# 0xSooki/stark-rs

Measured on AMD Instinct MI355X. Metric: ntt_field_elements_per_sec, higher is better.
Workload: dtype u32; 1 GPU; lde_2^22rows_x4cols_blowup8 (4 iNTT 2^22 + 4 coset NTT 2^25 per GPU per step); prime=469762049, parallelism=columns x1 (no collective)

## Files before the change

### stark_rs_amd/csrc/emu.cpp

```cpp
#include <array>
#include <vector>

#include "ntt_driver.h"
#include "lde_core.h"
#include "tables.h"
#include "proof_parse.h"

namespace {

std::vector<uint32_t> fill(const GeomSpec &s, const Fp &F) {
    std::vector<uint32_t> t((size_t)s.count << s.pair);
    for (uint32_t i = 0; i < s.count; i++) {
        const uint32_t v = geom_entry(s.c_m, s.q_m, i, s.stride, F);
        if (s.pair) { const Tw2 c = tw2_from_mont(v, F); t[2 * i] = c.w; t[2 * i + 1] = c.q; }
        else t[i] = v;
    }
    return t;
}

template <int LOGR, int LOGW, int KIND, int CAP> void emu_pass_cols(const PassArgs &a) {
    typedef NttPass<LOGR, LOGW, KIND, CAP> NP;
    constexpr bool LAST = KIND == PASS_LAST;
    const uint32_t NT = NP::NT;
    std::vector<uint32_t> tile(NP::R * NP::WP);
    std::vector<Tw2> tw(NP::R);
    std::vector<std::array<uint32_t, 16>> mw(NT), mq(NT), iw(NT), regs(NT);
    const bool twin = KIND == PASS_MID && (a.flags & NTT_TW_IN);
    auto r16 = [](std::array<uint32_t, 16> &x) -> uint32_t(&)[16] { return reinterpret_cast<uint32_t(&)[16]>(x); };
    for (uint32_t blk = 0; blk < a.n_tiles; blk++) {
        typename NP::TileId t = NP::tile_id(a, blk);
        for (uint32_t tid = 0; tid < NT; tid++) NP::load_tw(a, tw.data(), tid);
        for (uint32_t b = 0; b < a.batch; b++) {
            if (b % NP::COLS_PER_WG == 0)
                for (uint32_t tid = 0; tid < NT; tid++) {
                    NP::out_mul(a, t, tid, r16(mw[tid]), r16(mq[tid]));
                    if (twin) NP::in_mul(a, t, tid, r16(iw[tid]));
                }
            if (twin) {
                for (uint32_t tid = 0; tid < NT; tid++) {
                    NP::template load_regs<0, false>(a, t, b, r16(regs[tid]), tid);
                    for (int i = 0; i < 16; i++) regs[tid][i] = mont_mul(regs[tid][i], iw[tid][i], a.F);
                }
                for (uint32_t tid = 0; tid < NT; tid++) NP::template step0_regs<0>(a, r16(regs[tid]), tile.data(), tw.data(), tid);
            } else if (!LAST) {
#define ZCASE(Z)                                                                                                 \
    case Z:                                                                                                      \
        for (uint32_t tid = 0; tid < NT; tid++) NP::template load_regs<Z>(a, t, b, r16(regs[tid]), tid);         \
        for (uint32_t tid = 0; tid < NT; tid++) NP::template step0_regs<Z>(a, r16(regs[tid]), tile.data(), tw.data(), tid); \
        break;
                switch (a.zlog) { ZCASE(2) ZCASE(3) ZCASE(4) default: ZCASE(0) }
#undef ZCASE
            } else if (a.flags & NTT_LAST_DIRECT) {
                for (uint32_t tid = 0; tid < NT; tid++) NP::load_rows_direct(a, t, b, r16(regs[tid]), tid);
                for (uint32_t tid = 0; tid < NT; tid++) NP::step0_rows(a, r16(regs[tid]), tile.data(), tw.data(), tid);
            } else {
                for (uint32_t tid = 0; tid < NT; tid++) NP::load_rows(a, t, b, r16(regs[tid]), tid);
                for (uint32_t tid = 0; tid < NT; tid++) NP::rows_to_lds(r16(regs[tid]), tile.data(), tid);
                for (uint32_t tid = 0; tid < NT; tid++) NP::step0_lds(a, tile.data(), tw.data(), tid);
// ... 4 lines not shown
    }
}

int g_share_cols = 1;

template <int LOGR, int LOGW, int KIND, int CAP> void emu_pass(const PassArgs &a, uint32_t batch) {
    typedef NttPass<LOGR, LOGW, KIND, CAP> NP;
    constexpr bool LAST = KIND == PASS_LAST;
    if (g_share_cols && NP::share_cols(a, g_share_cols == 2 ? 0u : (uint32_t)NP::COLS_MIN_WGS)) return emu_pass_cols<LOGR, LOGW, KIND, CAP>(a);
    std::vector<uint32_t> tile(NP::R * NP::WP);
    std::vector<Tw2> tw(NP::R);
    for (uint32_t b = 0; b < batch; b++)
        for (uint32_t blk = 0; blk < a.n_tiles; blk++) {
            typename NP::TileId t = NP::tile_id(a, blk);
            const uint32_t NT = NP::NT;
            for (uint32_t tid = 0; tid < NT; tid++) NP::load_tw(a, tw.data(), tid);
            if (!LAST) {
                std::vector<std::array<uint32_t, 16>> regs(NT);
#define ZCASE(Z)                                                                                                           \
    case Z:                                                                                                                \
        for (uint32_t tid = 0; tid < NT; tid++) NP::template load_regs<Z>(a, t, b, reinterpret_cast<uint32_t(&)[16]>(regs[tid]), tid); \
        for (uint32_t tid = 0; tid < NT; tid++) NP::template step0_regs<Z>(a, reinterpret_cast<uint32_t(&)[16]>(regs[tid]), tile.data(), tw.data(), tid); \
        break;
                switch (a.zlog) { ZCASE(0) ZCASE(1) ZCASE(2) ZCASE(3) ZCASE(4) }
#undef ZCASE
            } else if (a.flags & NTT_LAST_DIRECT) {
                std::vector<std::array<uint32_t, 16>> regs(NT);
                for (uint32_t tid = 0; tid < NT; tid++) NP::load_rows_direct(a, t, b, reinterpret_cast<uint32_t(&)[16]>(regs[tid]), tid);
                for (uint32_t tid = 0; tid < NT; tid++) NP::step0_rows(a, reinterpret_cast<uint32_t(&)[16]>(regs[tid]), tile.data(), tw.data(), tid);
            } else {
// ... 578 lines not shown
```

### stark_rs_amd/csrc/internal.h

```cpp
#pragma once
#include <string.h>
#include <hip/hip_runtime.h>

#include <stdlib.h>

#include <string>
#include <vector>

#include "../../include/stark_mi.h"
#include "fri_plan.h"
#include "tables.h"
#include "transcript_core.h"

struct ScaleEntry {
    uint32_t c, q, L;
    uint32_t *lo, *hi;
    uint64_t epoch;
};

struct ProfRec {
    const char *name;
    hipEvent_t e0, e1;
    double bytes;
    double mixes;
// ... 12 lines not shown
    uint32_t *d_root_tab[32] = {};
    uint32_t *scratch = nullptr;
    size_t scratch_elems = 0;
    void *tmp[4] = {nullptr, nullptr, nullptr, nullptr};
    size_t tmp_bytes[4] = {0, 0, 0, 0};
    int *d_flag = nullptr;
    void *pin[2] = {nullptr, nullptr};
    hipEvent_t pin_ev[2] = {nullptr, nullptr};
    void *pin_out = nullptr;
    size_t pin_out_bytes = 0;
    std::string err;
    bool prof_on = false;
    char prof_only[56] = {0};
    bool copy_probe = false;
    bool ntt_share_cols = !(getenv("SMI_NTT_SHARE_COLS") && atoi(getenv("SMI_NTT_SHARE_COLS")) == 0);
    bool ntt_twin_regs = !(getenv("SMI_NTT_TWIN_REGS") && atoi(getenv("SMI_NTT_TWIN_REGS")) == 0);
    bool ntt_last_direct = !(getenv("SMI_NTT_LAST_DIRECT") && atoi(getenv("SMI_NTT_LAST_DIRECT")) == 0);
    int ntt_defer_tw = getenv("SMI_NTT_DEFER_TW") ? (atoi(getenv("SMI_NTT_DEFER_TW")) != 0) : 2;
    bool lde_two_pass = getenv("SMI_LDE_TWO_PASS") && atoi(getenv("SMI_LDE_TWO_PASS"));
    std::vector<ProfRec> prof;
    uint8_t *arena = nullptr;
    size_t arena_size = 0, arena_used = 0, arena_want = 0;
    std::vector<void *> arena_overflow;
};
int arena_reset(smi_ctx *ctx);
void *arena_alloc(smi_ctx *ctx, size_t bytes);

struct ProfScope {
    smi_ctx *ctx;
    ProfRec r;
    bool on;
// ... 211 lines not shown
```

### stark_rs_amd/csrc/ntt.hip

```cpp
#include "internal.h"
#include "ntt_driver.h"
#include "lde_core.h"

template <int LOGR, int LOGW, int KIND, int CAP>
__global__ __launch_bounds__(1 << (LOGR + LOGW - 4)) void ntt_pass_kernel(const PassArgs a) {
    typedef NttPass<LOGR, LOGW, KIND, CAP> NP;
    __shared__ uint32_t tile[NP::R * NP::WP];
    __shared__ Tw2 tw[NP::R];
    const uint32_t tid = threadIdx.x, batch = blockIdx.y;
    const typename NP::TileId t = NP::tile_id(a, blockIdx.x);
    NP::load_tw(a, tw, tid);
    uint32_t v[NP::V];
    if constexpr (KIND == PASS_FIRST) {
#define ZCASE(Z)                                         \
    case Z:                                              \
        NP::template load_regs<Z>(a, t, batch, v, tid);  \
        __syncthreads();       \
        NP::template step0_regs<Z>(a, v, tile, tw, tid); \
        break;
        switch (a.zlog) { ZCASE(2) ZCASE(3) ZCASE(4) default: ZCASE(0) }
#undef ZCASE
    } else if constexpr (KIND == PASS_MID) {
        NP::template load_regs<0>(a, t, batch, v, tid);
        __syncthreads();
        NP::template step0_regs<0>(a, v, tile, tw, tid);
    } else if (a.flags & NTT_LAST_DIRECT) {
        NP::load_rows_direct(a, t, batch, v, tid);
// ... 7 lines not shown
    }
    __syncthreads();
    if (NP::St::n == 3) {
        NP::step_mid(a, tile, tw, tid);
        __syncthreads();
    }
    NP::last_step_store(a, t, batch, tile, tw, tid);
}

#ifndef SMI_COLS_WAVES
#define SMI_COLS_WAVES(TILE_LOG, LOGR) ((TILE_LOG) >= 14 || (LOGR) >= 11 ? 4 : ((LOGR) == 10 ? 5 : 6))
#endif
#ifndef SMI_COLS_TWIN_WAVES
#define SMI_COLS_TWIN_WAVES 4
#endif
#ifndef SMI_COLS_TWIN_MQ
#define SMI_COLS_TWIN_MQ 1
#endif
#ifndef SMI_COLS_PREFETCH
#define SMI_COLS_PREFETCH 1
#endif
template <int LOGR, int LOGW, int KIND, int CAP, bool TWIN = false>
__global__ __launch_bounds__(1 << (LOGR + LOGW - 4), TWIN ? SMI_COLS_TWIN_WAVES : SMI_COLS_WAVES(LOGR + LOGW, LOGR)) void ntt_pass_cols_kernel(const PassArgs a) {
    typedef NttPass<LOGR, LOGW, KIND, CAP> NP;
    __shared__ uint32_t tile[NP::R * NP::WP];
    __shared__ Tw2 tw[NP::R];
    const uint32_t tid0 = threadIdx.x;
    const typename NP::TileId t = NP::tile_id(a, blockIdx.x);
    NP::load_tw(a, tw, tid0);
    constexpr bool MQ = !TWIN || SMI_COLS_TWIN_MQ;
    uint32_t mw[NP::V], mq[MQ ? NP::V : 1];
    NP::template out_mul<MQ>(a, t, tid0, mw, mq);
    uint32_t iw[TWIN ? NP::V : 1];
    if constexpr (TWIN) NP::in_mul(a, t, tid0, iw);
    const uint32_t col0 = blockIdx.y * NP::COLS_PER_WG, col1 = min(a.batch, col0 + (uint32_t)NP::COLS_PER_WG);
    if constexpr (SMI_COLS_PREFETCH && KIND == PASS_MID && LOGW == 5) {
        uint32_t v[NP::V];
        auto load = [&](uint32_t col) {
            uint32_t tid = tid0;
            asm volatile("" : "+v"(tid));
            NP::template load_regs<0, !TWIN>(a, t, col, v, tid);
        };
        load(col0);
        for (uint32_t batch = col0; batch < col1; batch++) {
            uint32_t tid = tid0;
            asm volatile("" : "+v"(tid));
            if constexpr (TWIN) {
#pragma unroll
                for (int i = 0; i < NP::V; i++) v[i] = mont_mul(v[i], iw[i], a.F);
            }
            __syncthreads();
            NP::template step0_regs<0>(a, v, tile, tw, tid);
            if (batch + 1 < col1) load(batch + 1);
            __syncthreads();
            if (NP::St::n == 3) {
                NP::step_mid(a, tile, tw, tid);
                __syncthreads();
            }
            NP::template last_step_store_mul<MQ>(a, t, batch, tile, tw, tid, mw, mq);
        }
        return;
    }
    for (uint32_t batch = col0; batch < col1; batch++) {
        uint32_t tid = tid0;
        asm volatile("" : "+v"(tid));
        uint32_t v[NP::V];
        static_assert(KIND != PASS_FIRST, "first passes keep one workgroup per (tile, column), NttPass::share_cols");
        if constexpr (KIND == PASS_MID) {
            NP::template load_regs<0, !TWIN>(a, t, batch, v, tid);
            if constexpr (TWIN) {
#pragma unroll
                for (int i = 0; i < NP::V; i++) v[i] = mont_mul(v[i], iw[i], a.F);
            }
            __syncthreads();
            NP::template step0_regs<0>(a, v, tile, tw, tid);
        } else if (a.flags & NTT_LAST_DIRECT) {
            NP::load_rows_direct(a, t, batch, v, tid);
            __syncthreads();
            NP::step0_rows(a, v, tile, tw, tid);
        } else {
            NP::load_rows(a, t, batch, v, tid);
            if (batch != col0) __syncthreads();
            NP::rows_to_lds(v, tile, tid);
            __syncthreads();
            NP::step0_lds(a, tile, tw, tid);
        }
        __syncthreads();
        if (NP::St::n == 3) {
            NP::step_mid(a, tile, tw, tid);
            __syncthreads();
        }
        NP::template last_step_store_mul<MQ>(a, t, batch, tile, tw, tid, mw, mq);
    }
}

template <int LOGR, int LOGW, int KIND>
__global__ __launch_bounds__(1 << (LOGR + LOGW - 4)) void ntt_copy_probe_kernel(const PassArgs a) {
    typedef NttPass<LOGR, LOGW, KIND, 4> NP;
    enum { NB = (NP::TILE / NP::RL) / NP::NT, KSTEP_LOG = LOGR - NP::SL };
    const uint32_t tid = threadIdx.x, batch = blockIdx.y;
    const typename NP::TileId t = NP::tile_id(a, blockIdx.x);
    uint32_t v[NP::V];
    const uint32_t lin = a.flags >> 30;
    const uint64_t lin_in = (uint64_t)batch * a.in_stride + (uint64_t)blockIdx.x * NP::TILE;
    const uint64_t lin_out = (uint64_t)batch * a.out_stride + (uint64_t)blockIdx.x * NP::TILE;
    if ((lin & 1u) && KIND != PASS_FIRST) {
#pragma unroll
        for (int i = 0; i < NP::V; i++) v[i] = ld32(a.in + lin_in, (uint32_t)i * NP::NT + tid);
    } else if constexpr (KIND == PASS_LAST) {
        if (a.flags & NTT_LAST_DIRECT) NP::load_rows_direct(a, t, batch, v, tid);
        else NP::load_rows(a, t, batch, v, tid);
    } else if constexpr (KIND == PASS_MID) {
        NP::template load_regs<0, false>(a, t, batch, v, tid);
    } else {
        switch (a.zlog) {
        case 2: NP::template load_regs<2>(a, t, batch, v, tid); break;
        case 3: NP::template load_regs<3>(a, t, batch, v, tid); break;
        case 4: NP::template load_regs<4>(a, t, batch, v, tid); break;
        default: NP::template load_regs<0>(a, t, batch, v, tid); break;
        }
    }
    if ((lin & 2u) && KIND != PASS_LAST) {
#pragma unroll
        for (int i = 0; i < NP::V; i++) st32(a.out + lin_out, (uint32_t)i * NP::NT + tid, v[i] + 1u);
        return;
    }
    uint32_t *out = a.out + (uint64_t)batch * a.out_stride + t.out_base;
    const uint32_t sh = KIND == PASS_LAST ? a.Sp : a.L - a.Sp - LOGR;
// ... 123 lines not shown
    widen_kernel<<<grid_for(n, 256), 256, 0, ctx->stream>>>(d_in, d_out, n);
    HIP_TRY(ctx, hipGetLastError());
    return SMI_OK;
}

namespace {
struct HipLauncher {
    smi_ctx *ctx;
    hipError_t err = hipSuccess;
    void small(const SmallArgs &a, uint32_t batch) {
        ProfScope ps(ctx, "ntt_small_kernel", (4.0 * a.n_in + 4.0 * (1ull << a.L)) * batch);
        ntt_small_kernel<<<batch, SMI_NTT_THREADS, 0, ctx->stream>>>(a);
        note();
    }
    template <int LR, int LW, int KIND, int CAP> void launch(const PassArgs &a) {
        if constexpr (KIND != PASS_FIRST) {
            if (ctx->ntt_share_cols && NttPass<LR, LW, KIND, CAP>::share_cols(a)) {
                const dim3 grid(a.n_tiles, NttPass<LR, LW, KIND, CAP>::col_groups(a));
                if (KIND == PASS_MID && (a.flags & NTT_TW_IN) && ctx->ntt_twin_regs)
                    ntt_pass_cols_kernel<LR, LW, KIND, CAP, KIND == PASS_MID><<<grid, 1 << (LR + LW - 4), 0, ctx->stream>>>(a);
                else
                    ntt_pass_cols_kernel<LR, LW, KIND, CAP><<<grid, 1 << (LR + LW - 4), 0, ctx->stream>>>(a);
                return;
            }
        }
        ntt_pass_kernel<LR, LW, KIND, CAP><<<dim3(a.n_tiles, a.batch), 1 << (LR + LW - 4), 0, ctx->stream>>>(a);
    }
    template <int LR, int LW> void launch_probe(int kind, const PassArgs &a0) {
        static const uint32_t lin = getenv("SMI_PROBE_LINEAR") ? (uint32_t)atoi(getenv("SMI_PROBE_LINEAR")) & 3u : 0u;
        PassArgs a = a0;
        a.flags |= lin << 30;
        const dim3 grid(a.n_tiles, a.batch);
        if (kind == PASS_FIRST) ntt_copy_probe_kernel<LR, LW, PASS_FIRST><<<grid, 1 << (LR + LW - 4), 0, ctx->stream>>>(a);
        else if (kind == PASS_MID) ntt_copy_probe_kernel<LR, LW, PASS_MID><<<grid, 1 << (LR + LW - 4), 0, ctx->stream>>>(a);
        else ntt_copy_probe_kernel<LR, LW, PASS_LAST><<<grid, 1 << (LR + LW - 4), 0, ctx->stream>>>(a);
    }
    template <int LR, int LW, int CAP> void launch_kind(int kind, const PassArgs &a) {
        if (kind == PASS_FIRST) launch<LR, LW, PASS_FIRST, CAP>(a);
        else if (kind == PASS_MID) launch<LR, LW, PASS_MID, CAP>(a);
        else launch<LR, LW, PASS_LAST, CAP>(a);
    }
// ... 186 lines not shown
```

### stark_rs_amd/csrc/ntt_core.h

```cpp
#pragma once
#include "field.h"

#if defined(SMI_EMU_CHECKS) && !defined(__HIP_DEVICE_COMPILE__)
#include <assert.h>
#define SMI_BOUND_CHECK(x, m, p) assert((m) <= 8 && (uint64_t)(x) < (uint64_t)((m) ? (m) : 1) * (p) && ((m) || (x) == 0))
#else
#define SMI_BOUND_CHECK(x, m, p) ((void)0)
#endif

#define SMI_TILE_LOG 12
#define SMI_TILE (1u << SMI_TILE_LOG)
#define SMI_NTT_THREADS 256
#define SMI_TW_LOG 12

struct alignas(8) Tw2 {
    uint32_t w, q;
};

struct NttTables {
    const Tw2 *tw10;
    const uint32_t *lo;
    const uint32_t *hi;
    uint32_t K, h;
};
// ... 68 lines not shown
#if defined(SMI_NTT_DBG_NOSTORE)
    if (v != 0xFFFFFFFFu) return;
#endif
#if defined(__HIP_DEVICE_COMPILE__) && SMI_NTT_NT
    __builtin_nontemporal_store(v, p);
#else
    *p = v;
#endif
}
SMI_HD Tw2 ld_tw(const Tw2 *base, uint32_t idx) { return *(const Tw2 *)((const char *)base + (size_t)(uint32_t)(idx << 3)); }

SMI_HD uint32_t shoup_mul(uint32_t a, const Tw2 &c, uint32_t p) {
    return a * c.w - umulhi32(a, c.q) * p;
}
SMI_HD uint32_t lz_canon(uint32_t a, uint32_t p) { return umin32(a, a - p); }

SMI_HD void lz_fold_m(uint32_t &x, int &m, uint32_t p) {
    if (m > 4) { x = umin32(x, x - 4u * p); m = 4; }
    else if (m > 2) { x = umin32(x, x - 2u * p); m = 2; }
}
SMI_HD void lz_fold_to2(uint32_t &x, int &m, uint32_t p) {
    lz_fold_m(x, m, p);
    lz_fold_m(x, m, p);
}
SMI_HD uint32_t lz_canon_m(uint32_t x, int m, uint32_t p) {
    lz_fold_to2(x, m, p);
    return m > 1 ? umin32(x, x - p) : x;
}

template <int S, int CAP, int Z = 0>
// ... 15 lines not shown
#pragma unroll
            for (int t = 0; t < 3; t++)
                if (m[i] + m[j] > CAP) {
                    if (m[i] >= m[j]) lz_fold_m(x[i], m[i], p);
                    else lz_fold_m(x[j], m[j], p);
                }
            const uint32_t u = x[i], v = x[j];
            const int ms = m[i] + m[j];
            SMI_BOUND_CHECK(u, m[i], p);
            SMI_BOUND_CHECK(v, m[j], p);
            x[i] = u + v;
            const uint32_t d = u - v + (uint32_t)m[j] * p;
            m[i] = ms;
            if (e) { x[j] = shoup_mul(d, cw[e << croot_shift], p); m[j] = 2; }
            else { x[j] = d; m[j] = ms; }
        }
    }
}

enum { PASS_FIRST = 0, PASS_MID = 1, PASS_LAST = 2 };
template <int LOGR, int LOGW, int KIND, int CAP> struct NttPass {
    static constexpr bool FIRST = KIND == PASS_FIRST, MID = KIND == PASS_MID, LAST = KIND == PASS_LAST;
    enum { TILE_LOG = LOGR + LOGW, TILE = 1 << TILE_LOG, NT = TILE / 16, R = 1 << LOGR, W = 1 << LOGW, WP = W + 1, V = 16 };
    typedef Steps<LOGR> St;
    enum { SL = St::n == 2 ? St::s1 : St::s2, RL = 1 << SL };

    struct TileId {
        uint64_t in_base, out_base;
        uint32_t b0;
    };
// ... 22 lines not shown
            t.b0 = k0_0;
            t.in_base = (((uint64_t)k0_0 << arest_log) + a_rest) << LOGR;
            t.out_base = ((uint64_t)rev << a.d0_log) + k0_0;
        }
        return t;
    }

    static SMI_HD void load_tw(const PassArgs &a, Tw2 *tw, uint32_t tid) {
#pragma unroll
        for (int i = 0; i < (R + NT - 1) / NT; i++) {
            uint32_t j = tid + i * NT;
            if (j < (uint32_t)R) tw[j] = a.T.tw10[j << (SMI_TW_LOG - LOGR)];
        }
    }

    template <int Z, bool TWIN = true> static SMI_HD void load_regs(const PassArgs &a, const TileId &t, uint32_t batch, uint32_t (&v)[V], uint32_t tid) {
        const uint32_t blog = a.L - a.Sp - LOGR, ablog = blog - a.shard_log;
        const uint32_t w = tid & (W - 1), j0 = tid >> LOGW;
        const uint32_t o0 = (j0 << ablog) + w;
        if constexpr (FIRST) {
            const uint32_t *col = a.in + (uint64_t)batch * a.in_stride;
            const uint32_t n0 = a.b_off + t.b0 + (j0 << blog) + w;
#pragma unroll
            for (int i = 0; i < V; i++) {
                if (i >= (V >> Z)) { v[i] = 0u; continue; }
                const uint32_t g = n0 + ((uint32_t)(i * (NT >> LOGW)) << blog);
                const uint32_t ga = t.b0 + o0 + ((uint32_t)(i * (NT >> LOGW)) << ablog);
                const uint32_t x = ld32(col, g < a.n_in ? ga : 0u);
                v[i] = g < a.n_in ? x : 0u;
            }
            if (a.flags & NTT_PRE_SCALE) {
                uint32_t sc = two_level(a.S.lo, a.S.hi, a.S.h, n0, a.F);
                const uint32_t rq = a.pre_ratio_m * a.F.pinv;
#pragma unroll
                for (int i = 0; i < (V >> Z); i++) {
                    v[i] = mont_mul(v[i], sc, a.F);
                    sc = mont_mul_c(sc, a.pre_ratio_m, rq, a.F);
                }
            }
        } else {
            const uint32_t *in = a.in + (uint64_t)batch * a.in_stride + t.in_base;
#pragma unroll
            for (int i = 0; i < V; i++) v[i] = ld32(in, o0 + ((uint32_t)(i * (NT >> LOGW)) << ablog));
            if (TWIN && (a.flags & NTT_TW_IN)) {
                const uint32_t sub = (uint32_t)(t.in_base >> (a.L - a.Sp)), k = sub & ((1u << a.prev_logr) - 1u);
                const uint32_t sh = a.T.K - (a.L - a.Sp + a.prev_logr);
                uint32_t cur = two_level(a.T.lo, a.T.hi, a.T.h, (k * ((j0 << blog) + t.b0 + w)) << sh, a.F);
                const uint32_t ratio = two_level(a.T.lo, a.T.hi, a.T.h, (k * ((uint32_t)(NT >> LOGW) << blog)) << sh, a.F);
                const uint32_t rq = ratio * a.F.pinv;
#pragma unroll
                for (int i = 0; i < V; i++) {
                    v[i] = mont_mul(v[i], cur, a.F);
                    if (i + 1 < V) cur = mont_mul_c(cur, ratio, rq, a.F);
                }
            }
        }
    }

    template <int Z> static SMI_HD void step0_regs(const PassArgs &a, uint32_t (&x)[V], uint32_t *tile, const Tw2 *tw, uint32_t tid) {
        enum { SUB = LOGR - 4 };
        const uint32_t w = tid & (W - 1), pos = tid >> LOGW;
        int m[16];
#pragma unroll
        for (int i = 0; i < 16; i++) m[i] = i < (V >> Z) ? 1 : 0;
        dft_regs<4, CAP, Z>(x, m, tw, LOGR - 4, a.F);
#pragma unroll
        for (int kk = 0; kk < 16; kk++) {
            uint32_t v = x[brev<4>(kk)];
            int mv = m[brev<4>(kk)];
            if (kk) v = shoup_mul(v, tw[(pos * kk) & (R - 1)], a.F.p);
            else lz_fold_to2(v, mv, a.F.p);
// ... 42 lines not shown
        direct_map(tid, pos, line);
        int m[16];
#pragma unroll
        for (int i = 0; i < 16; i++) m[i] = 1;
        dft_regs<4, CAP>(x, m, tw, LOGR - 4, a.F);
#pragma unroll
        for (int kk = 0; kk < 16; kk++) {
            uint32_t v = x[brev<4>(kk)];
            int mv = m[brev<4>(kk)];
            if (kk) v = shoup_mul(v, tw[(pos * kk) & (R - 1)], a.F.p);
            else lz_fold_to2(v, mv, a.F.p);
            tile[(pos + ((uint32_t)kk << SUB)) * WP + line] = v;
        }
    }

    template <int S, int MLOG, int MIN> static SMI_HD void step(const PassArgs &a, uint32_t *tile, const Tw2 *tw, uint32_t tid) {
        enum { r = 1 << S, SUB = MLOG - S, NB = (TILE / r) / NT };
#pragma unroll
        for (int bi = 0; bi < NB; bi++) {
            const uint32_t u = tid + bi * NT;
            const uint32_t w = u & (W - 1), ub = u >> LOGW;
            const uint32_t blk = ub >> SUB, pos = ub & ((1u << SUB) - 1u);
            const uint32_t base = (blk << MLOG) + pos;
            uint32_t x[r];
#pragma unroll
            for (int q = 0; q < r; q++) x[q] = tile[(base + ((uint32_t)q << SUB)) * WP + w];
            int m[r];
#pragma unroll
            for (int q = 0; q < r; q++) m[q] = MIN;
            dft_regs<S, CAP>(x, m, tw, LOGR - S, a.F);
#pragma unroll
            for (int kk = 0; kk < r; kk++) {
                uint32_t v = x[brev<S>(kk)];
                int mv = m[brev<S>(kk)];
                if (kk) v = shoup_mul(v, tw[((pos * kk) << (LOGR - MLOG)) & (R - 1)], a.F.p);
                else lz_fold_to2(v, mv, a.F.p);
                tile[(base + ((uint32_t)kk << SUB)) * WP + w] = v;
            }
        }
    }
    static SMI_HD void step0_lds(const PassArgs &a, uint32_t *tile, const Tw2 *tw, uint32_t tid) { step<4, LOGR, 1>(a, tile, tw, tid); }
    static SMI_HD void step_mid(const PassArgs &a, uint32_t *tile, const Tw2 *tw, uint32_t tid) {
        if constexpr (St::n == 3) step<St::s1, LOGR - St::s0, 2>(a, tile, tw, tid);
    }

    static SMI_HD uint32_t blk_to_k(uint32_t blk) {
        if (St::n == 2) return blk;
        const uint32_t k0 = blk >> St::s1, k1 = blk & ((1u << St::s1) - 1u);
        return k0 | (k1 << St::s0);
    }

    static SMI_HD void last_step_store(const PassArgs &a, const TileId &t, uint32_t batch, const uint32_t *tile, const Tw2 *tw,
                                       uint32_t tid) {
        enum { NB = (TILE / RL) / NT, KSTEP_LOG = LOGR - SL };
        uint32_t *out = a.out + (uint64_t)batch * a.out_stride + t.out_base;
        const uint32_t mlog = a.L - a.Sp, p = a.F.p;
        uint32_t base_run = 0, gs = 0, gq = 0, gbi = 0, gbq = 0;
        uint32_t sc_run = 0, rq = 0, rbq = 0;
        if (!LAST && !(a.flags & NTT_TW_SKIP)) {
            const uint32_t b = a.b_off + t.b0 + (tid & (W - 1)), sh = a.T.K - mlog;
            base_run = two_level(a.T.lo, a.T.hi, a.T.h, (b * blk_to_k(tid >> LOGW)) << sh, a.F);
            gs = two_level(a.T.lo, a.T.hi, a.T.h, (b << KSTEP_LOG) << sh, a.F);
            gq = gs * a.F.pinv;
            if (NB > 1) {
                gbi = two_level(a.T.lo, a.T.hi, a.T.h, (b << SL) << sh, a.F);
                gbq = gbi * a.F.pinv;
            }
        }
        if (LAST && (a.flags & NTT_POST_SCALE)) {
            sc_run = two_level(a.S.lo, a.S.hi, a.S.h, (uint32_t)t.out_base + (blk_to_k(tid >> LOGW) << a.Sp) + (tid & (W - 1)), a.F);
            rq = a.post_ratio_m * a.F.pinv;
            rbq = a.post_bi_ratio_m * a.F.pinv;
        }
#pragma unroll
        for (int bi = 0; bi < NB; bi++) {
            const uint32_t u = tid + bi * NT;
            const uint32_t w = u & (W - 1), blk = u >> LOGW;
            uint32_t x[RL];
#pragma unroll
            for (int q = 0; q < RL; q++) x[q] = tile[(blk * RL + q) * WP + w];
            int m[RL];
#pragma unroll
            for (int q = 0; q < RL; q++) m[q] = 2;
            dft_regs<SL, CAP>(x, m, tw, LOGR - SL, a.F);
            const uint32_t kbase = blk_to_k(blk);
            if constexpr (!LAST) {
                const uint32_t blog = mlog - LOGR - a.shard_log;
                const uint32_t o0 = (kbase << blog) + w;
                {
                    if (a.flags & NTT_TW_SKIP) {
#pragma unroll
                        for (int kk = 0; kk < RL; kk++) {
                            SMI_BOUND_CHECK(x[brev<SL>(kk)], m[brev<SL>(kk)], p);
                            st32(out, o0 + ((uint32_t)kk << (KSTEP_LOG + blog)), x[brev<SL>(kk)]);
                        }
                        continue;
                    }
                    uint32_t cur = base_run;
                    if (bi + 1 < NB) base_run = mont_mul_c(base_run, gbi, gbq, a.F);
#pragma unroll
// ... 14 lines not shown
                    }
                } else {
#pragma unroll
                    for (int kk = 0; kk < RL; kk++) st32(out, o0 + ((uint32_t)kk << (KSTEP_LOG + a.Sp)), lz_canon_m(x[brev<SL>(kk)], m[brev<SL>(kk)], p));
                }
            }
        }
    }

    static SMI_HD bool has_out_mul(const PassArgs &a) { return LAST ? (a.flags & NTT_POST_SCALE) != 0 : !(a.flags & NTT_TW_SKIP); }
    enum { COLS_PER_WG = SMI_COLS_PER_WG, COLS_MIN_WGS = SMI_COLS_MIN_WGS };
    static SMI_HD uint32_t col_groups(const PassArgs &a) { return (a.batch + COLS_PER_WG - 1) / COLS_PER_WG; }
    static SMI_HD bool share_cols(const PassArgs &a, uint32_t min_wgs = COLS_MIN_WGS) {
        return !FIRST && a.batch > 1 && has_out_mul(a) && (uint64_t)a.n_tiles * col_groups(a) >= min_wgs;
    }
    template <bool MQ = true>
    static SMI_HD void out_mul(const PassArgs &a, const TileId &t, uint32_t tid, uint32_t (&mw)[V], uint32_t (&mq)[MQ ? V : 1]) {
        enum { NB = (TILE / RL) / NT, KSTEP_LOG = LOGR - SL };
        const uint32_t w = tid & (W - 1), kb0 = blk_to_k(tid >> LOGW);
        uint32_t run, step, step_bi = 0;
        if (!LAST) {
            const uint32_t b = a.b_off + t.b0 + w, sh = a.T.K - (a.L - a.Sp);
            run = two_level(a.T.lo, a.T.hi, a.T.h, (b * kb0) << sh, a.F);
            step = two_level(a.T.lo, a.T.hi, a.T.h, (b << KSTEP_LOG) << sh, a.F);
            if (NB > 1) step_bi = two_level(a.T.lo, a.T.hi, a.T.h, (b << SL) << sh, a.F);
        } else {
            run = two_level(a.S.lo, a.S.hi, a.S.h, (uint32_t)t.out_base + (kb0 << a.Sp) + w, a.F);
            step = a.post_ratio_m;
            step_bi = a.post_bi_ratio_m;
        }
        const uint32_t sq = step * a.F.pinv, bq = step_bi * a.F.pinv;
#pragma unroll
        for (int bi = 0; bi < NB; bi++) {
            uint32_t cur = run;
            if (bi + 1 < NB) run = mont_mul_c(run, step_bi, bq, a.F);
#pragma unroll
            for (int kk = 0; kk < RL; kk++) {
                mw[bi * RL + kk] = cur;
                if constexpr (MQ) mq[bi * RL + kk] = cur * a.F.pinv;
                if (kk + 1 < RL) cur = mont_mul_c(cur, step, sq, a.F);
            }
        }
    }
    static SMI_HD void in_mul(const PassArgs &a, const TileId &t, uint32_t tid, uint32_t (&iw)[V]) {
        const uint32_t blog = a.L - a.Sp - LOGR;
        const uint32_t w = tid & (W - 1), j0 = tid >> LOGW;
        const uint32_t sub = (uint32_t)(t.in_base >> (a.L - a.Sp)), k = sub & ((1u << a.prev_logr) - 1u);
        const uint32_t sh = a.T.K - (a.L - a.Sp + a.prev_logr);
        uint32_t cur = two_level(a.T.lo, a.T.hi, a.T.h, (k * ((j0 << blog) + t.b0 + w)) << sh, a.F);
        const uint32_t ratio = two_level(a.T.lo, a.T.hi, a.T.h, (k * ((uint32_t)(NT >> LOGW) << blog)) << sh, a.F);
        const uint32_t rq = ratio * a.F.pinv;
#pragma unroll
        for (int i = 0; i < V; i++) {
            iw[i] = cur;
            if (i + 1 < V) cur = mont_mul_c(cur, ratio, rq, a.F);
        }
    }
    template <bool MQ = true>
    static SMI_HD void last_step_store_mul(const PassArgs &a, const TileId &t, uint32_t batch, const uint32_t *tile, const Tw2 *tw,
                                           uint32_t tid, const uint32_t (&mw)[V], const uint32_t (&mq)[MQ ? V : 1]) {
        enum { NB = (TILE / RL) / NT, KSTEP_LOG = LOGR - SL };
        uint32_t *out = a.out + (uint64_t)batch * a.out_stride + t.out_base;
        const uint32_t olog = LAST ? a.Sp : a.L - a.Sp - LOGR - a.shard_log;
#pragma unroll
        for (int bi = 0; bi < NB; bi++) {
            const uint32_t u = tid + bi * NT;
            const uint32_t w = u & (W - 1), blk = u >> LOGW;
            uint32_t x[RL];
#pragma unroll
            for (int q = 0; q < RL; q++) x[q] = tile[(blk * RL + q) * WP + w];
            int m[RL];
#pragma unroll
            for (int q = 0; q < RL; q++) m[q] = 2;
            dft_regs<SL, CAP>(x, m, tw, LOGR - SL, a.F);
            const uint32_t o0 = (blk_to_k(blk) << olog) + w;
#pragma unroll
            for (int kk = 0; kk < RL; kk++)
                if constexpr (MQ) st32(out, o0 + ((uint32_t)kk << (KSTEP_LOG + olog)), mont_mul_c(x[brev<SL>(kk)], mw[bi * RL + kk], mq[bi * RL + kk], a.F));
                else st32(out, o0 + ((uint32_t)kk << (KSTEP_LOG + olog)), mont_mul(x[brev<SL>(kk)], mw[bi * RL + kk], a.F));
        }
    }
};

struct SmallArgs {
    const uint32_t *in;
    uint32_t *out;
    uint64_t in_stride, out_stride;
    Fp F;
    NttTables T;
    ScaleTables S;
    uint32_t L, n_in, flags;
};
struct NttSmall {
    static SMI_HD uint32_t at(uint32_t i) { return i + (i >> 6); }
// ... 51 lines not shown
```

Measured before the change: 229.9 billion field-elements/s.

## Fold inter-pass twiddles into coset butterfly nodes for middle NTT passes

Middle passes that used to multiply every loaded element by a per-element input twiddle (in_mul) now run a coset-style DIT butterfly. It uses per-tile node twiddles that already include the previous pass's twist. The output exponent is adjusted so the remaining twist is absorbed into the existing out_mul. This removes one Montgomery multiply per element and the in_mul register arrays. In exchange, a per-tile node table is computed in shared memory with two_level lookups, and each butterfly stage uses distinct per-position twiddles.

```diff
diff --git a/stark_rs_amd/csrc/emu.cpp b/stark_rs_amd/csrc/emu.cpp
--- a/stark_rs_amd/csrc/emu.cpp
+++ b/stark_rs_amd/csrc/emu.cpp
@@ -24,24 +24,24 @@
     const uint32_t NT = NP::NT;
     std::vector<uint32_t> tile(NP::R * NP::WP);
     std::vector<Tw2> tw(NP::R);
-    std::vector<std::array<uint32_t, 16>> mw(NT), mq(NT), iw(NT), regs(NT);
+    std::vector<std::array<uint32_t, 16>> mw(NT), mq(NT), regs(NT);
     const bool twin = KIND == PASS_MID && (a.flags & NTT_TW_IN);
     auto r16 = [](std::array<uint32_t, 16> &x) -> uint32_t(&)[16] { return reinterpret_cast<uint32_t(&)[16]>(x); };
     for (uint32_t blk = 0; blk < a.n_tiles; blk++) {
         typename NP::TileId t = NP::tile_id(a, blk);
-        for (uint32_t tid = 0; tid < NT; tid++) NP::load_tw(a, tw.data(), tid);
+        for (uint32_t tid = 0; tid < NT; tid++) {
+            if (twin) NP::load_nodes(a, t, tw.data(), tid);
+            else NP::load_tw(a, tw.data(), tid);
+        }
         for (uint32_t b = 0; b < a.batch; b++) {
             if (b % NP::COLS_PER_WG == 0)
-                for (uint32_t tid = 0; tid < NT; tid++) {
-                    NP::out_mul(a, t, tid, r16(mw[tid]), r16(mq[tid]));
-                    if (twin) NP::in_mul(a, t, tid, r16(iw[tid]));
-                }
+                for (uint32_t tid = 0; tid < NT; tid++) NP::out_mul(a, t, tid, r16(mw[tid]), r16(mq[tid]));
             if (twin) {
-                for (uint32_t tid = 0; tid < NT; tid++) {
-                    NP::template load_regs<0, false>(a, t, b, r16(regs[tid]), tid);
-                    for (int i = 0; i < 16; i++) regs[tid][i] = mont_mul(regs[tid][i], iw[tid][i], a.F);
-                }
-                for (uint32_t tid = 0; tid < NT; tid++) NP::template step0_regs<0>(a, r16(regs[tid]), tile.data(), tw.data(), tid);
+                for (uint32_t tid = 0; tid < NT; tid++) NP::template load_regs<0>(a, t, b, r16(regs[tid]), tid);
+                for (uint32_t tid = 0; tid < NT; tid++) NP::step0_coset(a, r16(regs[tid]), tile.data(), tw.data(), tid);
+                for (uint32_t tid = 0; tid < NT; tid++) NP::template step_mid<true>(a, tile.data(), tw.data(), tid);
+                for (uint32_t tid = 0; tid < NT; tid++) NP::template last_step_store_mul<true>(a, t, b, tile.data(), tw.data(), tid, r16(mw[tid]), r16(mq[tid]));
+                continue;
             } else if (!LAST) {
 #define ZCASE(Z)                                                                                                 \
     case Z:                                                                                                      \
@@ -76,6 +76,15 @@
         for (uint32_t blk = 0; blk < a.n_tiles; blk++) {
             typename NP::TileId t = NP::tile_id(a, blk);
             const uint32_t NT = NP::NT;
+            if (KIND == PASS_MID && (a.flags & NTT_TW_IN)) {
+                std::vector<std::array<uint32_t, 16>> regs(NT);
+                for (uint32_t tid = 0; tid < NT; tid++) NP::load_nodes(a, t, tw.data(), tid);
+                for (uint32_t tid = 0; tid < NT; tid++) NP::template load_regs<0>(a, t, b, reinterpret_cast<uint32_t(&)[16]>(regs[tid]), tid);
+                for (uint32_t tid = 0; tid < NT; tid++) NP::step0_coset(a, reinterpret_cast<uint32_t(&)[16]>(regs[tid]), tile.data(), tw.data(), tid);
+                for (uint32_t tid = 0; tid < NT; tid++) NP::template step_mid<true>(a, tile.data(), tw.data(), tid);
+                for (uint32_t tid = 0; tid < NT; tid++) NP::template last_step_store<true>(a, t, b, tile.data(), tw.data(), tid);
+                continue;
+            }
             for (uint32_t tid = 0; tid < NT; tid++) NP::load_tw(a, tw.data(), tid);
             if (!LAST) {
                 std::vector<std::array<uint32_t, 16>> regs(NT);
diff --git a/stark_rs_amd/csrc/internal.h b/stark_rs_amd/csrc/internal.h
--- a/stark_rs_amd/csrc/internal.h
+++ b/stark_rs_amd/csrc/internal.h
@@ -50,7 +50,6 @@
     char prof_only[56] = {0};
     bool copy_probe = false;
     bool ntt_share_cols = !(getenv("SMI_NTT_SHARE_COLS") && atoi(getenv("SMI_NTT_SHARE_COLS")) == 0);
-    bool ntt_twin_regs = !(getenv("SMI_NTT_TWIN_REGS") && atoi(getenv("SMI_NTT_TWIN_REGS")) == 0);
     bool ntt_last_direct = !(getenv("SMI_NTT_LAST_DIRECT") && atoi(getenv("SMI_NTT_LAST_DIRECT")) == 0);
     int ntt_defer_tw = getenv("SMI_NTT_DEFER_TW") ? (atoi(getenv("SMI_NTT_DEFER_TW")) != 0) : 2;
     bool lde_two_pass = getenv("SMI_LDE_TWO_PASS") && atoi(getenv("SMI_LDE_TWO_PASS"));
diff --git a/stark_rs_amd/csrc/ntt.hip b/stark_rs_amd/csrc/ntt.hip
--- a/stark_rs_amd/csrc/ntt.hip
+++ b/stark_rs_amd/csrc/ntt.hip
@@ -2,15 +2,29 @@
 #include "ntt_driver.h"
 #include "lde_core.h"
 
-template <int LOGR, int LOGW, int KIND, int CAP>
+template <int LOGR, int LOGW, int KIND, int CAP, bool TWIN = false>
 __global__ __launch_bounds__(1 << (LOGR + LOGW - 4)) void ntt_pass_kernel(const PassArgs a) {
     typedef NttPass<LOGR, LOGW, KIND, CAP> NP;
     __shared__ uint32_t tile[NP::R * NP::WP];
     __shared__ Tw2 tw[NP::R];
     const uint32_t tid = threadIdx.x, batch = blockIdx.y;
     const typename NP::TileId t = NP::tile_id(a, blockIdx.x);
+    uint32_t v[NP::V];
+    if constexpr (TWIN) {
+        static_assert(KIND == PASS_MID, "only a middle pass takes over the first pass's twiddles");
+        NP::load_nodes(a, t, tw, tid);
+        NP::template load_regs<0>(a, t, batch, v, tid);
+        __syncthreads();
+        NP::step0_coset(a, v, tile, tw, tid);
+        __syncthreads();
+        if (NP::St::n == 3) {
+            NP::template step_mid<true>(a, tile, tw, tid);
+            __syncthreads();
+        }
+        NP::template last_step_store<true>(a, t, batch, tile, tw, tid);
+        return;
+    }
     NP::load_tw(a, tw, tid);
-    uint32_t v[NP::V];
     if constexpr (KIND == PASS_FIRST) {
 #define ZCASE(Z)                                         \
     case Z:                                              \
@@ -48,9 +62,6 @@
 #ifndef SMI_COLS_TWIN_WAVES
 #define SMI_COLS_TWIN_WAVES 4
 #endif
-#ifndef SMI_COLS_TWIN_MQ
-#define SMI_COLS_TWIN_MQ 1
-#endif
 #ifndef SMI_COLS_PREFETCH
 #define SMI_COLS_PREFETCH 1
 #endif
@@ -61,37 +72,33 @@
     __shared__ Tw2 tw[NP::R];
     const uint32_t tid0 = threadIdx.x;
     const typename NP::TileId t = NP::tile_id(a, blockIdx.x);
-    NP::load_tw(a, tw, tid0);
-    constexpr bool MQ = !TWIN || SMI_COLS_TWIN_MQ;
-    uint32_t mw[NP::V], mq[MQ ? NP::V : 1];
-    NP::template out_mul<MQ>(a, t, tid0, mw, mq);
-    uint32_t iw[TWIN ? NP::V : 1];
-    if constexpr (TWIN) NP::in_mul(a, t, tid0, iw);
+    static_assert(!TWIN || KIND == PASS_MID, "only a middle pass takes over the first pass's twiddles");
+    if constexpr (TWIN) NP::load_nodes(a, t, tw, tid0);
+    else NP::load_tw(a, tw, tid0);
+    uint32_t mw[NP::V], mq[NP::V];
+    NP::out_mul(a, t, tid0, mw, mq);
     const uint32_t col0 = blockIdx.y * NP::COLS_PER_WG, col1 = min(a.batch, col0 + (uint32_t)NP::COLS_PER_WG);
     if constexpr (SMI_COLS_PREFETCH && KIND == PASS_MID && LOGW == 5) {
         uint32_t v[NP::V];
         auto load = [&](uint32_t col) {
             uint32_t tid = tid0;
             asm volatile("" : "+v"(tid));
-            NP::template load_regs<0, !TWIN>(a, t, col, v, tid);
+            NP::template load_regs<0>(a, t, col, v, tid);
         };
         load(col0);
         for (uint32_t batch = col0; batch < col1; batch++) {
             uint32_t tid = tid0;
             asm volatile("" : "+v"(tid));
-            if constexpr (TWIN) {
-#pragma unroll
-                for (int i = 0; i < NP::V; i++) v[i] = mont_mul(v[i], iw[i], a.F);
-            }
-            __syncthreads();
-            NP::template step0_regs<0>(a, v, tile, tw, tid);
+            __syncthreads();
+            if constexpr (TWIN) NP::step0_coset(a, v, tile, tw, tid);
+            else NP::template step0_regs<0>(a, v, tile, tw, tid);
             if (batch + 1 < col1) load(batch + 1);
             __syncthreads();
             if (NP::St::n == 3) {
-                NP::step_mid(a, tile, tw, tid);
+                NP::template step_mid<TWIN>(a, tile, tw, tid);
                 __syncthreads();
             }
-            NP::template last_step_store_mul<MQ>(a, t, batch, tile, tw, tid, mw, mq);
+            NP::template last_step_store_mul<TWIN>(a, t, batch, tile, tw, tid, mw, mq);
         }
         return;
     }
@@ -101,13 +108,10 @@
         uint32_t v[NP::V];
         static_assert(KIND != PASS_FIRST, "first passes keep one workgroup per (tile, column), NttPass::share_cols");
         if constexpr (KIND == PASS_MID) {
-            NP::template load_regs<0, !TWIN>(a, t, batch, v, tid);
-            if constexpr (TWIN) {
-#pragma unroll
-                for (int i = 0; i < NP::V; i++) v[i] = mont_mul(v[i], iw[i], a.F);
-            }
-            __syncthreads();
-            NP::template step0_regs<0>(a, v, tile, tw, tid);
+            NP::template load_regs<0>(a, t, batch, v, tid);
+            __syncthreads();
+            if constexpr (TWIN) NP::step0_coset(a, v, tile, tw, tid);
+            else NP::template step0_regs<0>(a, v, tile, tw, tid);
         } else if (a.flags & NTT_LAST_DIRECT) {
             NP::load_rows_direct(a, t, batch, v, tid);
             __syncthreads();
@@ -121,10 +125,10 @@
         }
         __syncthreads();
         if (NP::St::n == 3) {
-            NP::step_mid(a, tile, tw, tid);
-            __syncthreads();
-        }
-        NP::template last_step_store_mul<MQ>(a, t, batch, tile, tw, tid, mw, mq);
+            NP::template step_mid<TWIN>(a, tile, tw, tid);
+            __syncthreads();
+        }
+        NP::template last_step_store_mul<TWIN>(a, t, batch, tile, tw, tid, mw, mq);
     }
 }
 
@@ -145,7 +149,7 @@
         if (a.flags & NTT_LAST_DIRECT) NP::load_rows_direct(a, t, batch, v, tid);
         else NP::load_rows(a, t, batch, v, tid);
     } else if constexpr (KIND == PASS_MID) {
-        NP::template load_regs<0, false>(a, t, batch, v, tid);
+        NP::template load_regs<0>(a, t, batch, v, tid);
     } else {
         switch (a.zlog) {
         case 2: NP::template load_regs<2>(a, t, batch, v, tid); break;
@@ -299,17 +303,17 @@
         note();
     }
     template <int LR, int LW, int KIND, int CAP> void launch(const PassArgs &a) {
+        const bool twin = KIND == PASS_MID && (a.flags & NTT_TW_IN);
         if constexpr (KIND != PASS_FIRST) {
             if (ctx->ntt_share_cols && NttPass<LR, LW, KIND, CAP>::share_cols(a)) {
                 const dim3 grid(a.n_tiles, NttPass<LR, LW, KIND, CAP>::col_groups(a));
-                if (KIND == PASS_MID && (a.flags & NTT_TW_IN) && ctx->ntt_twin_regs)
-                    ntt_pass_cols_kernel<LR, LW, KIND, CAP, KIND == PASS_MID><<<grid, 1 << (LR + LW - 4), 0, ctx->stream>>>(a);
-                else
-                    ntt_pass_cols_kernel<LR, LW, KIND, CAP><<<grid, 1 << (LR + LW - 4), 0, ctx->stream>>>(a);
+                if (twin) ntt_pass_cols_kernel<LR, LW, KIND, CAP, KIND == PASS_MID><<<grid, 1 << (LR + LW - 4), 0, ctx->stream>>>(a);
+                else ntt_pass_cols_kernel<LR, LW, KIND, CAP><<<grid, 1 << (LR + LW - 4), 0, ctx->stream>>>(a);
                 return;
             }
         }
-        ntt_pass_kernel<LR, LW, KIND, CAP><<<dim3(a.n_tiles, a.batch), 1 << (LR + LW - 4), 0, ctx->stream>>>(a);
+        if (twin) ntt_pass_kernel<LR, LW, KIND, CAP, KIND == PASS_MID><<<dim3(a.n_tiles, a.batch), 1 << (LR + LW - 4), 0, ctx->stream>>>(a);
+        else ntt_pass_kernel<LR, LW, KIND, CAP><<<dim3(a.n_tiles, a.batch), 1 << (LR + LW - 4), 0, ctx->stream>>>(a);
     }
     template <int LR, int LW> void launch_probe(int kind, const PassArgs &a0) {
         static const uint32_t lin = getenv("SMI_PROBE_LINEAR") ? (uint32_t)atoi(getenv("SMI_PROBE_LINEAR")) & 3u : 0u;
diff --git a/stark_rs_amd/csrc/ntt_core.h b/stark_rs_amd/csrc/ntt_core.h
--- a/stark_rs_amd/csrc/ntt_core.h
+++ b/stark_rs_amd/csrc/ntt_core.h
@@ -106,6 +106,28 @@
     return a * c.w - umulhi32(a, c.q) * p;
 }
 SMI_HD uint32_t lz_canon(uint32_t a, uint32_t p) { return umin32(a, a - p); }
+SMI_HD Tw2 tw2_of_mont(uint32_t v_m, const Fp &F) { return Tw2{mont_mul(v_m, 1u, F), (0u - v_m) * F.pinv}; }
+SMI_HD uint32_t uniform32(uint32_t v) {
+#if defined(__HIP_DEVICE_COMPILE__)
+    return __builtin_amdgcn_readfirstlane(v);
+#else
+    return v;
+#endif
+}
+SMI_HD uint32_t ilog2_32(uint32_t x) {
+#if defined(__HIP_DEVICE_COMPILE__)
+    return 31u - (uint32_t)__clz((int)x);
+#else
+    uint32_t l = 0;
+    while (x >>= 1) l++;
+    return l;
+#endif
+}
+SMI_HD constexpr uint32_t brev_n(uint32_t x, int s) {
+    uint32_t r = 0;
+    for (int i = 0; i < s; i++) r |= ((x >> i) & 1u) << (s - 1 - i);
+    return r;
+}
 
 SMI_HD void lz_fold_m(uint32_t &x, int &m, uint32_t p) {
     if (m > 4) { x = umin32(x, x - 4u * p); m = 4; }
@@ -151,6 +173,28 @@
             m[i] = ms;
             if (e) { x[j] = shoup_mul(d, cw[e << croot_shift], p); m[j] = 2; }
             else { x[j] = d; m[j] = ms; }
+        }
+    }
+}
+
+template <int S, int CAP>
+SMI_HD void coset_regs(uint32_t (&x)[1 << S], int (&m)[1 << S], const Tw2 (&c)[(1 << S) - 1], uint32_t p) {
+#pragma unroll
+    for (int s = 0; s < S; s++) {
+        const int half = (1 << S) >> (s + 1);
+#pragma unroll
+        for (int i = 0; i < (1 << S); i++) {
+            if (i & half) continue;
+            const int j = i | half;
+#pragma unroll
+            for (int t = 0; t < 2; t++)
+                if (m[i] + 2 > CAP) lz_fold_m(x[i], m[i], p);
+            SMI_BOUND_CHECK(x[i], m[i], p);
+            SMI_BOUND_CHECK(x[j], m[j], p);
+            const uint32_t u = x[i], t = shoup_mul(x[j], c[(1 << s) - 1 + (i >> (S - s))], p);
+            x[i] = u + t;
+            x[j] = u - t + 2u * p;
+            m[i] = m[j] = m[i] + 2;
         }
     }
 }
@@ -203,7 +247,24 @@
         }
     }
 
-    template <int Z, bool TWIN = true> static SMI_HD void load_regs(const PassArgs &a, const TileId &t, uint32_t batch, uint32_t (&v)[V], uint32_t tid) {
+    static SMI_HD uint32_t prev_k(const PassArgs &a, const TileId &t) {
+        return (uint32_t)(t.in_base >> (a.L - a.Sp)) & ((1u << a.prev_logr) - 1u);
+    }
+    static SMI_HD uint32_t node(uint32_t l, uint32_t kappa) { return (1u << l) - 1u + kappa; }
+    static SMI_HD void load_nodes(const PassArgs &a, const TileId &t, Tw2 *tw, uint32_t tid) {
+        const uint32_t k = prev_k(a, t);
+#pragma unroll
+        for (int i = 0; i < (R + NT - 1) / NT; i++) {
+            const uint32_t j = tid + i * NT + 1u;
+            if (j < (uint32_t)R) {
+                const uint32_t l = ilog2_32(j), kappa = j - (1u << l);
+                const uint32_t e = (k + (kappa << a.prev_logr)) << (a.T.K - a.prev_logr - l - 1u);
+                tw[j - 1u] = tw2_of_mont(two_level(a.T.lo, a.T.hi, a.T.h, e, a.F), a.F);
+            }
+        }
+    }
+
+    template <int Z> static SMI_HD void load_regs(const PassArgs &a, const TileId &t, uint32_t batch, uint32_t (&v)[V], uint32_t tid) {
         const uint32_t blog = a.L - a.Sp - LOGR, ablog = blog - a.shard_log;
         const uint32_t w = tid & (W - 1), j0 = tid >> LOGW;
         const uint32_t o0 = (j0 << ablog) + w;
@@ -231,19 +292,32 @@
             const uint32_t *in = a.in + (uint64_t)batch * a.in_stride + t.in_base;
 #pragma unroll
             for (int i = 0; i < V; i++) v[i] = ld32(in, o0 + ((uint32_t)(i * (NT >> LOGW)) << ablog));
-            if (TWIN && (a.flags & NTT_TW_IN)) {
-                const uint32_t sub = (uint32_t)(t.in_base >> (a.L - a.Sp)), k = sub & ((1u << a.prev_logr) - 1u);
-                const uint32_t sh = a.T.K - (a.L - a.Sp + a.prev_logr);
-                uint32_t cur = two_level(a.T.lo, a.T.hi, a.T.h, (k * ((j0 << blog) + t.b0 + w)) << sh, a.F);
-                const uint32_t ratio = two_level(a.T.lo, a.T.hi, a.T.h, (k * ((uint32_t)(NT >> LOGW) << blog)) << sh, a.F);
-                const uint32_t rq = ratio * a.F.pinv;
-#pragma unroll
-                for (int i = 0; i < V; i++) {
-                    v[i] = mont_mul(v[i], cur, a.F);
-                    if (i + 1 < V) cur = mont_mul_c(cur, ratio, rq, a.F);
-                }
-            }
-        }
+        }
+    }
+
+    static SMI_HD void step0_coset(const PassArgs &a, uint32_t (&x)[V], uint32_t *tile, const Tw2 *nodes, uint32_t tid) {
+        enum { SUB = LOGR - 4 };
+        const uint32_t w = tid & (W - 1), pos = tid >> LOGW;
+        Tw2 c[15];
+#pragma unroll
+        for (int s = 0; s < 4; s++)
+#pragma unroll
+            for (int tq = 0; tq < (1 << s); tq++) {
+                const Tw2 n = nodes[node(s, brev_n(tq, s))];
+                c[(1 << s) - 1 + tq] = Tw2{uniform32(n.w), uniform32(n.q)};
+            }
+        int m[16];
+#pragma unroll
+        for (int i = 0; i < 16; i++) m[i] = CAP;
+        coset_regs<4, CAP>(x, m, c, a.F.p);
+#pragma unroll
+        for (int kk = 0; kk < 16; kk++) tile[(pos + ((uint32_t)kk << SUB)) * WP + w] = x[brev<4>(kk)];
+    }
+    template <int S, int L0> static SMI_HD void step_nodes(const Tw2 *nodes, uint32_t kb, Tw2 (&c)[(1 << S) - 1]) {
+#pragma unroll
+        for (int s = 0; s < S; s++)
+#pragma unroll
+            for (int tq = 0; tq < (1 << s); tq++) c[(1 << s) - 1 + tq] = nodes[node(L0 + s, kb + (brev_n(tq, s) << L0))];
     }
 
     template <int Z> static SMI_HD void step0_regs(const PassArgs &a, uint32_t (&x)[V], uint32_t *tile, const Tw2 *tw, uint32_t tid) {
@@ -316,7 +390,7 @@
         }
     }
 
-    template <int S, int MLOG, int MIN> static SMI_HD void step(const PassArgs &a, uint32_t *tile, const Tw2 *tw, uint32_t tid) {
+    template <int S, int MLOG, int MIN, bool CS = false> static SMI_HD void step(const PassArgs &a, uint32_t *tile, const Tw2 *tw, uint32_t tid) {
         enum { r = 1 << S, SUB = MLOG - S, NB = (TILE / r) / NT };
 #pragma unroll
         for (int bi = 0; bi < NB; bi++) {
@@ -328,6 +402,16 @@
 #pragma unroll
             for (int q = 0; q < r; q++) x[q] = tile[(base + ((uint32_t)q << SUB)) * WP + w];
             int m[r];
+            if constexpr (CS) {
+                Tw2 c[r - 1];
+                step_nodes<S, LOGR - MLOG>(tw, blk, c);
+#pragma unroll
+                for (int q = 0; q < r; q++) m[q] = CAP;
+                coset_regs<S, CAP>(x, m, c, a.F.p);
+#pragma unroll
+                for (int kk = 0; kk < r; kk++) tile[(base + ((uint32_t)kk << SUB)) * WP + w] = x[brev<S>(kk)];
+                continue;
+            }
 #pragma unroll
             for (int q = 0; q < r; q++) m[q] = MIN;
             dft_regs<S, CAP>(x, m, tw, LOGR - S, a.F);
@@ -342,8 +426,8 @@
         }
     }
     static SMI_HD void step0_lds(const PassArgs &a, uint32_t *tile, const Tw2 *tw, uint32_t tid) { step<4, LOGR, 1>(a, tile, tw, tid); }
-    static SMI_HD void step_mid(const PassArgs &a, uint32_t *tile, const Tw2 *tw, uint32_t tid) {
-        if constexpr (St::n == 3) step<St::s1, LOGR - St::s0, 2>(a, tile, tw, tid);
+    template <bool CS = false> static SMI_HD void step_mid(const PassArgs &a, uint32_t *tile, const Tw2 *tw, uint32_t tid) {
+        if constexpr (St::n == 3) step<St::s1, LOGR - St::s0, 2, CS>(a, tile, tw, tid);
     }
 
     static SMI_HD uint32_t blk_to_k(uint32_t blk) {
@@ -352,6 +436,25 @@
         return k0 | (k1 << St::s0);
     }
 
+    static SMI_HD uint32_t out_exp(const PassArgs &a, const TileId &t, uint32_t b, uint32_t kb) {
+        const uint32_t sh = a.T.K - (a.L - a.Sp);
+        if (!MID || !(a.flags & NTT_TW_IN)) return (b * kb) << sh;
+        return (b * ((kb << a.prev_logr) + prev_k(a, t))) << (sh - a.prev_logr);
+    }
+    template <bool CS> static SMI_HD void last_regs(const PassArgs &a, uint32_t (&x)[RL], int (&m)[RL], const Tw2 *tw, uint32_t kbase) {
+        if constexpr (CS) {
+            Tw2 c[RL - 1];
+            step_nodes<SL, LOGR - SL>(tw, kbase, c);
+#pragma unroll
+            for (int q = 0; q < RL; q++) m[q] = CAP;
+            coset_regs<SL, CAP>(x, m, c, a.F.p);
+        } else {
+#pragma unroll
+            for (int q = 0; q < RL; q++) m[q] = 2;
+            dft_regs<SL, CAP>(x, m, tw, LOGR - SL, a.F);
+        }
+    }
+    template <bool CS = false>
     static SMI_HD void last_step_store(const PassArgs &a, const TileId &t, uint32_t batch, const uint32_t *tile, const Tw2 *tw,
                                        uint32_t tid) {
         enum { NB = (TILE / RL) / NT, KSTEP_LOG = LOGR - SL };
@@ -361,7 +464,7 @@
         uint32_t sc_run = 0, rq = 0, rbq = 0;
         if (!LAST && !(a.flags & NTT_TW_SKIP)) {
             const uint32_t b = a.b_off + t.b0 + (tid & (W - 1)), sh = a.T.K - mlog;
-            base_run = two_level(a.T.lo, a.T.hi, a.T.h, (b * blk_to_k(tid >> LOGW)) << sh, a.F);
+            base_run = two_level(a.T.lo, a.T.hi, a.T.h, out_exp(a, t, b, blk_to_k(tid >> LOGW)), a.F);
             gs = two_level(a.T.lo, a.T.hi, a.T.h, (b << KSTEP_LOG) << sh, a.F);
             gq = gs * a.F.pinv;
             if (NB > 1) {
@@ -382,10 +485,8 @@
 #pragma unroll
             for (int q = 0; q < RL; q++) x[q] = tile[(blk * RL + q) * WP + w];
             int m[RL];
-#pragma unroll
-            for (int q = 0; q < RL; q++) m[q] = 2;
-            dft_regs<SL, CAP>(x, m, tw, LOGR - SL, a.F);
             const uint32_t kbase = blk_to_k(blk);
+            last_regs<CS>(a, x, m, tw, kbase);
             if constexpr (!LAST) {
                 const uint32_t blog = mlog - LOGR - a.shard_log;
                 const uint32_t o0 = (kbase << blog) + w;
@@ -430,14 +531,13 @@
     static SMI_HD bool share_cols(const PassArgs &a, uint32_t min_wgs = COLS_MIN_WGS) {
         return !FIRST && a.batch > 1 && has_out_mul(a) && (uint64_t)a.n_tiles * col_groups(a) >= min_wgs;
     }
-    template <bool MQ = true>
-    static SMI_HD void out_mul(const PassArgs &a, const TileId &t, uint32_t tid, uint32_t (&mw)[V], uint32_t (&mq)[MQ ? V : 1]) {
+    static SMI_HD void out_mul(const PassArgs &a, const TileId &t, uint32_t tid, uint32_t (&mw)[V], uint32_t (&mq)[V]) {
         enum { NB = (TILE / RL) / NT, KSTEP_LOG = LOGR - SL };
         const uint32_t w = tid & (W - 1), kb0 = blk_to_k(tid >> LOGW);
         uint32_t run, step, step_bi = 0;
         if (!LAST) {
             const uint32_t b = a.b_off + t.b0 + w, sh = a.T.K - (a.L - a.Sp);
-            run = two_level(a.T.lo, a.T.hi, a.T.h, (b * kb0) << sh, a.F);
+            run = two_level(a.T.lo, a.T.hi, a.T.h, out_exp(a, t, b, kb0), a.F);
             step = two_level(a.T.lo, a.T.hi, a.T.h, (b << KSTEP_LOG) << sh, a.F);
             if (NB > 1) step_bi = two_level(a.T.lo, a.T.hi, a.T.h, (b << SL) << sh, a.F);
         } else {
@@ -453,28 +553,14 @@
 #pragma unroll
             for (int kk = 0; kk < RL; kk++) {
                 mw[bi * RL + kk] = cur;
-                if constexpr (MQ) mq[bi * RL + kk] = cur * a.F.pinv;
+                mq[bi * RL + kk] = cur * a.F.pinv;
                 if (kk + 1 < RL) cur = mont_mul_c(cur, step, sq, a.F);
             }
         }
     }
-    static SMI_HD void in_mul(const PassArgs &a, const TileId &t, uint32_t tid, uint32_t (&iw)[V]) {
-        const uint32_t blog = a.L - a.Sp - LOGR;
-        const uint32_t w = tid & (W - 1), j0 = tid >> LOGW;
-        const uint32_t sub = (uint32_t)(t.in_base >> (a.L - a.Sp)), k = sub & ((1u << a.prev_logr) - 1u);
-        const uint32_t sh = a.T.K - (a.L - a.Sp + a.prev_logr);
-        uint32_t cur = two_level(a.T.lo, a.T.hi, a.T.h, (k * ((j0 << blog) + t.b0 + w)) << sh, a.F);
-        const uint32_t ratio = two_level(a.T.lo, a.T.hi, a.T.h, (k * ((uint32_t)(NT >> LOGW) << blog)) << sh, a.F);
-        const uint32_t rq = ratio * a.F.pinv;
-#pragma unroll
-        for (int i = 0; i < V; i++) {
-            iw[i] = cur;
-            if (i + 1 < V) cur = mont_mul_c(cur, ratio, rq, a.F);
-        }
-    }
-    template <bool MQ = true>
+    template <bool CS = false>
     static SMI_HD void last_step_store_mul(const PassArgs &a, const TileId &t, uint32_t batch, const uint32_t *tile, const Tw2 *tw,
-                                           uint32_t tid, const uint32_t (&mw)[V], const uint32_t (&mq)[MQ ? V : 1]) {
+                                           uint32_t tid, const uint32_t (&mw)[V], const uint32_t (&mq)[V]) {
         enum { NB = (TILE / RL) / NT, KSTEP_LOG = LOGR - SL };
         uint32_t *out = a.out + (uint64_t)batch * a.out_stride + t.out_base;
         const uint32_t olog = LAST ? a.Sp : a.L - a.Sp - LOGR - a.shard_log;
@@ -486,14 +572,11 @@
 #pragma unroll
             for (int q = 0; q < RL; q++) x[q] = tile[(blk * RL + q) * WP + w];
             int m[RL];
-#pragma unroll
-            for (int q = 0; q < RL; q++) m[q] = 2;
-            dft_regs<SL, CAP>(x, m, tw, LOGR - SL, a.F);
+            last_regs<CS>(a, x, m, tw, blk_to_k(blk));
             const uint32_t o0 = (blk_to_k(blk) << olog) + w;
 #pragma unroll
             for (int kk = 0; kk < RL; kk++)
-                if constexpr (MQ) st32(out, o0 + ((uint32_t)kk << (KSTEP_LOG + olog)), mont_mul_c(x[brev<SL>(kk)], mw[bi * RL + kk], mq[bi * RL + kk], a.F));
-                else st32(out, o0 + ((uint32_t)kk << (KSTEP_LOG + olog)), mont_mul(x[brev<SL>(kk)], mw[bi * RL + kk], a.F));
+                st32(out, o0 + ((uint32_t)kk << (KSTEP_LOG + olog)), mont_mul_c(x[brev<SL>(kk)], mw[bi * RL + kk], mq[bi * RL + kk], a.F));
         }
     }
 };
```

After: 236.0 billion field-elements/s, median of 6. 2.6% higher.
